# debbiemarkslab/BEAR

Hardware: AMD Instinct MI355X
Metric: k-mer contexts/sec (DM-marginal+grad h), k=13 (higher is better)
Workload: dtype f64

## Files before the change

### bear_amd/csrc/bear_hip.hip

```cpp
#include "bear_host.h"
#include "kernels_finalize.h"
#include "kernels_rows.h"
#include "kernels_sorted.h"
#include "kernels_plan.h"
#include "kernels_synth.h"
#include "kernels_refmix.h"
#include "kernels_mixplan.h"
#include "kernels_sample.h"
#include "kernels_refplan.h"

#ifdef PLN_STAMPS
#define PLN_DBG_ARG , ws->dbg
#else
#define PLN_DBG_ARG
#endif

extern "C" {

int bear_abi_version(void) { return BEAR_ABI_VERSION; }

const char *bear_strerror(int status) {
  switch (status) {
    case BEAR_OK: return "ok";
    case BEAR_ERR_INVALID_ARG: return "invalid argument (null or misaligned pointer, bad flag)";
// ... 360 lines not shown

static int plan_count_live_rows(bear_plan *p, const plan_scan &sc) {
  unsigned long long h_hist[SRT_NKEY];
  HIP_TRY(hipMemcpy(h_hist, p->hist, sizeof(h_hist), hipMemcpyDeviceToHost));
  unsigned long long live_rows = sc.heavy[1];
  for (int k = 0; k < SRT_NKEY; ++k) live_rows += h_hist[k];
  p->n_live_rows = live_rows;
  return BEAR_OK;
}

static int plan_build(const bear_ws *ws, bear_plan *p) {
  plan_scan sc;
  plan_cut cut;
  int st = plan_scan_table(ws, p, sc);
  if (st != BEAR_OK) return st;
  const char *cut_env = getenv("BEAR_PLAN_CUT");
  st = cut_env && cut_env[0] == 'h' ? cut_on_host(p, sc, cut) : cut_on_device(p, sc, cut);
  if (st != BEAR_OK) return st;
  p->tiles = cut.tiles.release();
  p->n_tiles = cut.n_tiles;
  const uint64_t stream_bytes = cut.off16 * 16 + 1024;
  const uint64_t live_bytes = p->ncol == 5 ? sizeof(uint16_t) * PLN_LIVE_STRIDE * (p->n_tiles + 1) : 0;
  st = plan_fill(ws, p, sc, stream_bytes);
  if (st == BEAR_OK && live_bytes) st = plan_live_lists(ws, p, live_bytes);
  if (st != BEAR_OK) return st;
  HIP_TRY(hipDeviceSynchronize());
  unsigned long long h_used[3] = {0, 0, 0};
  HIP_TRY(hipMemcpy(h_used, sc.cnt.get() + 3, sizeof(h_used), hipMemcpyDeviceToHost));
  for (int k = 0; k < 3; ++k) p->n_heavy[k] = h_used[k];
  st = plan_order_lists(p);
  p->n_live_rows = p->n_rows;
  if (st == BEAR_OK && p->ncol == 5) st = plan_count_live_rows(p, sc);
  p->bytes = stream_bytes + live_bytes + sizeof(pln_tile) * p->n_tiles + sizeof(pln_heavy_col) * sc.heavy[0] +
             sizeof(pln_heavy_row) * sc.heavy[1] + sizeof(uint64_t) * sc.heavy[2];
  return st;
}

int bear_plan_create(bear_ws *ws, const uint32_t *counts, uint64_t n_rows, int ncol, bear_plan **out) {
  if (!out) return BEAR_ERR_INVALID_ARG;
  *out = nullptr;
  int st = check_ws(ws);
  if (st != BEAR_OK) return st;
  if ((ncol != 4 && ncol != 5) || (n_rows && !counts) || misaligned(counts)) return BEAR_ERR_INVALID_ARG;
  plan_guard p(new (std::nothrow) bear_plan());
  if (!p) return BEAR_ERR_NOMEM;
  memset(p.get(), 0, sizeof(bear_plan));
  p->device = ws->device;
  p->ncol = ncol;
  p->n_rows = n_rows;
  p->counts = counts;
  HIP_TRY(hipMalloc(&p->hist, sizeof(unsigned long long) * PLAN_HIST_WORDS));
  HIP_TRY(hipMemset(p->hist, 0, sizeof(unsigned long long) * PLAN_HIST_WORDS));
  if (n_rows) st = plan_build(ws, p.get());
  if (st == BEAR_OK) *out = p.release();
  return st;
}

int bear_plan_destroy(bear_plan *plan) {
  if (!plan) return BEAR_OK;
  int prev = 0;
  (void)hipGetDevice(&prev);
  (void)hipSetDevice(plan->device);
  plan_free(plan);
  (void)hipSetDevice(prev);
  return BEAR_OK;
}

uint64_t bear_plan_bytes(const bear_plan *plan) { return plan ? plan->bytes : 0; }

int bear_plan_create_auto(bear_ws *ws, const uint32_t *counts, uint64_t n_rows, int *rowwise, bear_plan **out) {
  if (rowwise) *rowwise = 0;
  int st = bear_plan_create(ws, counts, n_rows, 5, out);
  if (st != BEAR_OK) return st;
  bear_plan *p = *out;
  const double cells = p->count_total[1], listed = (double)p->n_heavy[0];
  if (!(cells > 0.0) || listed * 2.0 <= cells) return BEAR_OK;
  plan_drop_sorted(p);
  plan_drop_live(p);
  p->ncol = PLAN_ROWS;
  if (rowwise) *rowwise = 1;
  return BEAR_OK;
}
static int launch_prior_rows(bear_ws *ws, const bear_plan *plan, const double *prior, const bear_params &prm, const double *theta,
                             int train_ar, double *out, double *grad_prior, hipStream_t s) {
  const int grid = grid_dense(ws, plan->n_rows);
  const double2 *lt = reinterpret_cast<const double2 *>(ws->logtab);
  const bear_step_io io = ws_io(ws, theta, BEAR_THETA_NET, out);
#define ROWS_LAUNCH(AR, GRAD) \
  hipLaunchKernelGGL((dm_prior_rows_kernel<AR, GRAD>), dim3(grid), dim3(BEAR_THREADS), 0, s, plan->counts, prior, plan->n_rows, prm, grad_prior, lt, \
                     ws->partials, io)
  BEAR_DISPATCH_2(train_ar, grad_prior, ROWS_LAUNCH);
#undef ROWS_LAUNCH
  HIP_TRY(hipGetLastError());
  return BEAR_OK;
}

uint64_t bear_plan_tile_count(const bear_plan *plan) { return plan ? plan->n_tiles : 0; }

int bear_plan_tile_info(const bear_plan *plan, uint64_t first, uint64_t count, uint64_t *row0, uint32_t *rows, uint32_t *items,
                        uint64_t *stream_offset) {
  if (!plan || first + count > plan->n_tiles || (count && (!row0 || !rows || !items || !stream_offset))) return BEAR_ERR_INVALID_ARG;
  if (!count) return BEAR_OK;
  std::vector<pln_tile> h(count);
  int prev = 0;
  (void)hipGetDevice(&prev);
  (void)hipSetDevice(plan->device);
  const hipError_t e = hipMemcpy(h.data(), plan->tiles + first, sizeof(pln_tile) * count, hipMemcpyDeviceToHost);
  (void)hipSetDevice(prev);
  HIP_TRY(e);
  for (uint64_t k = 0; k < count; ++k) {
    row0[k] = h[k].row0;
    rows[k] = h[k].rows_items >> 16;
    items[k] = h[k].rows_items & 0xffffu;
    stream_offset[k] = (uint64_t)h[k].off16 * 16;
  }
  return BEAR_OK;
}

int bear_plan_create_ref(bear_ws *ws, const uint32_t *train, const uint32_t *ref, uint64_t n_rows, bear_plan **out) {
  if (!out) return BEAR_ERR_INVALID_ARG;
  *out = nullptr;
  if ((n_rows && !ref) || misaligned(ref)) return BEAR_ERR_INVALID_ARG;
  bear_plan *created = nullptr;
  int st = bear_plan_create(ws, train, n_rows, 4, &created);
  if (st != BEAR_OK) return st;
  plan_guard p(created);
  p->ref = ref;
  if (p->count_total[1] > 0.0 && (double)p->n_heavy[0] * 2.0 > p->count_total[1]) {
    plan_drop_sorted(p.get());
    p->rows_ref = 1;
    *out = p.release();
    return BEAR_OK;
  }
  HIP_TRY(hipMalloc(&p->hist0_base, sizeof(unsigned long long) * 72));
  unsigned long long *d_meta = p->hist0_base;
  HIP_TRY(hipMemset(d_meta, 0, sizeof(unsigned long long) * 72));
  HIP_TRY(hipMalloc(&p->sum0, sizeof(double)));
  HIP_TRY(hipMemset(p->sum0, 0, sizeof(double)));
  unsigned long long h_meta[72];
  memset(h_meta, 0, sizeof(h_meta));
  const int grid = grid_capped((n_rows + 1023) / 1024, (uint64_t)ws->num_cu * 8);
  if (n_rows) {
    hipLaunchKernelGGL(rpl_build_kernel, dim3(grid), dim3(256), 0, 0, train, ref, n_rows, 0, d_meta, d_meta + 32, d_meta + 64, p->sum0,
                       static_cast<rpl_item *>(nullptr), static_cast<uint32_t *>(nullptr));
    HIP_TRY(hipGetLastError());
    HIP_TRY(hipMemcpy(h_meta, d_meta, sizeof(h_meta), hipMemcpyDeviceToHost));
  }
  unsigned long long run = 0, cur[RPL_NKEY];
  for (int k = 0; k < RPL_NKEY; ++k) {
    cur[k] = run;
    run += h_meta[k];
  }
  p->n_ref_items = run;
  p->n_heavy0 = h_meta[64];
  if (run) HIP_TRY(hipMalloc(&p->ref_items, sizeof(rpl_item) * run));
  if (p->n_heavy0) HIP_TRY(hipMalloc(&p->heavy0, sizeof(uint32_t) * p->n_heavy0));
  HIP_TRY(hipMemcpy(d_meta, cur, sizeof(cur), hipMemcpyHostToDevice));
  HIP_TRY(hipMemset(d_meta + 64, 0, sizeof(unsigned long long)));
  if (n_rows && (run || p->n_heavy0)) {
    hipLaunchKernelGGL(rpl_build_kernel, dim3(grid), dim3(256), 0, 0, train, ref, n_rows, 1, d_meta, d_meta + 32, d_meta + 64, p->sum0,
                       p->ref_items, p->heavy0);
    HIP_TRY(hipGetLastError());
  }
  HIP_TRY(hipDeviceSynchronize());
#ifdef BEAR_DET_BUILD
  for (int k = 0; k < RPL_NKEY && st == BEAR_OK; ++k) st = bear_canonical_order(p->ref_items + cur[k], h_meta[k], 16, 0);
  if (st == BEAR_OK) st = bear_canonical_order(p->heavy0, p->n_heavy0, 4, 0);
  if (st != BEAR_OK) return st;
#endif
  p->hist0 = d_meta + 32;
  p->bytes += sizeof(rpl_item) * p->n_ref_items + sizeof(uint32_t) * p->n_heavy0 + sizeof(unsigned long long) * 72;
  *out = p.release();
  return BEAR_OK;
}

static int launch_prior_plan(bear_ws *ws, const bear_plan *plan, const double *prior, uint64_t n_rows, const bear_params &prm,
                             const double *theta, int train_ar, int prior_normalized, double *out, hipStream_t s) {
  const int grid = grid_plan(ws, plan->n_tiles);
  const double2 *lt = reinterpret_cast<const double2 *>(ws->logtab);
  const bear_step_io io = ws_io(ws, theta, BEAR_THETA_NET, out);
  if (train_ar)
    hipLaunchKernelGGL((dm_prior_plan_kernel<true, true>), dim3(grid), dim3(PLN_THREADS), sizeof(pln_lds_n), s, prior, n_rows, prm,
                       plan_view(plan), lt, ws->partials, io PLN_DBG_ARG);
  else if (prior_normalized)
    hipLaunchKernelGGL((dm_prior_plan_kernel<true, false>), dim3(grid), dim3(PLN_THREADS), sizeof(pln_lds_n), s, prior, n_rows, prm,
                       plan_view(plan), lt, ws->partials, io PLN_DBG_ARG);
  else
    hipLaunchKernelGGL((dm_prior_plan_kernel<false, false>), dim3(grid), dim3(PLN_THREADS), sizeof(pln_lds_n), s, prior, n_rows, prm,
                       plan_view(plan), lt, ws->partials, io PLN_DBG_ARG);
  HIP_TRY(hipGetLastError());
  return BEAR_OK;
}

int bear_dm_prior_plan_f64(bear_ws *ws, const bear_plan *plan, const uint32_t *counts, const double *prior,
                           uint64_t n_rows, double h_signed, double eps, int train_ar, int prior_normalized,
                           double *out, void *stream) {
  int st = check_ws(ws);
  if (st != BEAR_OK) return st;
  if (!plan || !out || (n_rows && (!counts || !prior))) return BEAR_ERR_INVALID_ARG;
  if (check_plan_step(ws, plan, counts, n_rows, 5, true) != BEAR_OK || misaligned(prior) || misaligned8(out)) return BEAR_ERR_INVALID_ARG;
  const bear_params prm = params_net(h_signed, eps);
  if (plan_is_rows(plan)) return launch_prior_rows(ws, plan, prior, prm, nullptr, train_ar, out, nullptr, static_cast<hipStream_t>(stream));
  return launch_prior_plan(ws, plan, prior, n_rows, prm, nullptr, train_ar, prior_normalized, out, static_cast<hipStream_t>(stream));
}

int launch_prior_plan_grad(bear_ws *ws, const bear_plan *plan, const double *prior, const bear_params &prm,
                                  const double *theta, int train_ar, int prior_normalized, double *out, double *grad_prior,
                                  hipStream_t s) {
  const int grid = grid_plan(ws, plan->n_tiles);
  const double2 *lt = reinterpret_cast<const double2 *>(ws->logtab);
  const pln_view pv = plan_view(plan);
  const bear_step_io io = ws_io(ws, theta, BEAR_THETA_NET, out);
  if (train_ar)
    hipLaunchKernelGGL((dm_prior_plan_grad_kernel<true, true>), dim3(grid), dim3(PLN_THREADS), sizeof(pln_lds_g), s, prior, prm, pv, lt,
                       grad_prior, ws->partials, io);
  else if (prior_normalized)
    hipLaunchKernelGGL(dm_prior_plan_grad_inplace_kernel, dim3(grid), dim3(PLN_THREADS), sizeof(pln_lds_gi), s, prior, prm, pv, lt,
                       grad_prior, ws->partials, io);
  else
    hipLaunchKernelGGL((dm_prior_plan_grad_kernel<false, false>), dim3(grid), dim3(PLN_THREADS), sizeof(pln_lds_g), s, prior, prm, pv, lt,
                       grad_prior, ws->partials, io);
  HIP_TRY(hipGetLastError());
  auto fixup_grid = [&](uint64_t nh) { return grid_capped((nh + 255) / 256, (uint64_t)ws->num_cu * 8); };
#define FIXUP(NORM, AR, ROWS, N) \
  hipLaunchKernelGGL((dm_prior_grad_fixup_kernel<NORM, AR, ROWS>), dim3(fixup_grid(N)), dim3(256), 0, s, prior, prm, pv, lt, grad_prior, io)
  if (pv.n_heavy_row && !train_ar) {
    if (prior_normalized) FIXUP(true, false, true, pv.n_heavy_row);
    else FIXUP(false, false, true, pv.n_heavy_row);
  }
  if (pv.n_heavy_col) {
    if (train_ar) FIXUP(true, true, false, pv.n_heavy_col);
    else if (prior_normalized) FIXUP(true, false, false, pv.n_heavy_col);
    else FIXUP(false, false, false, pv.n_heavy_col);
  }
#undef FIXUP
  HIP_TRY(hipGetLastError());
  return BEAR_OK;
}

int bear_dm_prior_plan_grad_f64(bear_ws *ws, const bear_plan *plan, const uint32_t *counts, const double *prior,
                                uint64_t n_rows, double h_signed, double eps, int train_ar, int prior_normalized,
                                double *out, double *grad_prior, void *stream) {
  int st = check_ws(ws);
  if (st != BEAR_OK) return st;
  if (!plan || !out || !grad_prior || (n_rows && (!counts || !prior))) return BEAR_ERR_INVALID_ARG;
  if (check_plan_step(ws, plan, counts, n_rows, 5, true) != BEAR_OK) return BEAR_ERR_INVALID_ARG;
  if (misaligned(prior) || misaligned(grad_prior) || misaligned8(out)) return BEAR_ERR_INVALID_ARG;
  const bear_params prm = params_net(h_signed, eps);
  if (plan_is_rows(plan)) return launch_prior_rows(ws, plan, prior, prm, nullptr, train_ar, out, grad_prior, static_cast<hipStream_t>(stream));
  return launch_prior_plan_grad(ws, plan, prior, prm, nullptr, train_ar, prior_normalized, out, grad_prior,
                                static_cast<hipStream_t>(stream));
}

int bear_dm_prior_plan_dev_f64(bear_ws *ws, const bear_plan *plan, const uint32_t *counts, const double *prior, uint64_t n_rows,
                               const double *h_signed_dev, double eps, int train_ar, int prior_normalized, double *out,
                               double *grad_prior, void *stream) {
  int st = check_ws(ws);
  if (st != BEAR_OK) return st;
  if (!plan || !out || !h_signed_dev || (n_rows && (!counts || !prior))) return BEAR_ERR_INVALID_ARG;
  if (check_plan_step(ws, plan, counts, n_rows, 5, true) != BEAR_OK) return BEAR_ERR_INVALID_ARG;
  if (misaligned(prior) || misaligned(grad_prior) || misaligned8(out)) return BEAR_ERR_INVALID_ARG;
  hipStream_t s = static_cast<hipStream_t>(stream);
  const bear_params only_eps = params_eps(eps);
  if (plan_is_rows(plan)) return launch_prior_rows(ws, plan, prior, only_eps, h_signed_dev, train_ar, out, grad_prior, s);
  if (grad_prior) return launch_prior_plan_grad(ws, plan, prior, only_eps, h_signed_dev, train_ar, prior_normalized, out, grad_prior, s);
  return launch_prior_plan(ws, plan, prior, n_rows, only_eps, h_signed_dev, train_ar, prior_normalized, out, s);
}

int bear_dm_refmix_plan_grad_f64(bear_ws *ws, const bear_plan *plan, const uint32_t *counts, const double *net_rows,
                                 const double *ref_rows, uint64_t n_rows, const double *h_signed_dev, const double *tau_signed_dev,
                                 const double *net_weight_signed_dev, double eps, int train_ar, double *out, double *grad_net_rows,
                                 void *stream) {
  int st = check_ws(ws);
  if (st != BEAR_OK) return st;
  if (!plan || !out || !h_signed_dev || !tau_signed_dev || !net_weight_signed_dev) return BEAR_ERR_INVALID_ARG;
  if (n_rows && (!counts || !net_rows || !ref_rows || !grad_net_rows)) return BEAR_ERR_INVALID_ARG;
  if (check_plan_step(ws, plan, counts, n_rows, 5) != BEAR_OK) return BEAR_ERR_INVALID_ARG;
  if (misaligned(net_rows) || misaligned(ref_rows) || misaligned(grad_net_rows) || misaligned8(out) || misaligned8(h_signed_dev) ||
      misaligned8(tau_signed_dev) || misaligned8(net_weight_signed_dev) || !(eps >= 0.0))
    return BEAR_ERR_INVALID_ARG;
  hipStream_t s = static_cast<hipStream_t>(stream);
  const int grid = grid_plan(ws, plan->n_tiles);
  const double2 *lt = reinterpret_cast<const double2 *>(ws->logtab);
  const pln_view pv = plan_view(plan);
  const bear_step_io io = ws_io(ws, nullptr, BEAR_THETA_REF, out);
#define MIX_LAUNCH(AR)                                                                                                            \
  hipLaunchKernelGGL(dm_refmix_plan_grad_kernel<AR>, dim3(grid), dim3(PLN_THREADS), sizeof(pln_lds_g), s, net_rows, ref_rows, \
                     h_signed_dev, tau_signed_dev, net_weight_signed_dev, eps, pv, lt, grad_net_rows, ws->partials, io)
  BEAR_DISPATCH_1(train_ar, MIX_LAUNCH);
#undef MIX_LAUNCH
  HIP_TRY(hipGetLastError());
  if (pv.n_heavy_col + pv.n_heavy_row) {
    const uint64_t nh = pv.n_heavy_col + pv.n_heavy_row;
    const int g2 = grid_capped((nh + 255) / 256, (uint64_t)ws->num_cu * 4);
#define MIX_FIXUP(AR)                                                                                                      \
  hipLaunchKernelGGL(dm_refmix_fixup_kernel<AR>, dim3(g2), dim3(256), 0, s, net_rows, ref_rows, h_signed_dev, tau_signed_dev, \
                     net_weight_signed_dev, eps, pv, lt, grad_net_rows)
    BEAR_DISPATCH_1(train_ar, MIX_FIXUP);
#undef MIX_FIXUP
    HIP_TRY(hipGetLastError());
  }
  return BEAR_OK;
}


static int launch_ref_plan(bear_ws *ws, const bear_plan *plan, const uint32_t *ref, uint64_t n_rows, const bear_params &prm,
                           const double *theta, int train_ar, double *out, hipStream_t s, const bear_apply_io &apply = NO_APPLY) {
  const double2 *lt = reinterpret_cast<const double2 *>(ws->logtab);
  const bear_step_io io = ws_io(ws, theta, BEAR_THETA_REF, out);
  int grid;
  if (plan->rows_ref) {
    if (plan->ref != ref) return BEAR_ERR_INVALID_ARG;
    grid = grid_dense(ws, n_rows);
#define REF_ROWS(AR) \
  hipLaunchKernelGGL(dm_ref_rows_kernel<AR>, dim3(grid), dim3(BEAR_THREADS), 0, s, plan->counts, ref, n_rows, prm, lt, ws->partials, io, apply)
    BEAR_DISPATCH_1(train_ar, REF_ROWS);
#undef REF_ROWS
  } else if (plan->ref) {
    if (plan->ref != ref) return BEAR_ERR_INVALID_ARG;
    rpl_view rv;
    rv.items = plan->ref_items;
    rv.n_items = plan->n_ref_items;
    rv.hist0 = plan->hist0;
    rv.heavy0 = plan->heavy0;
    rv.n_heavy0 = plan->n_heavy0;
    rv.sum0 = plan->sum0;
    const uint64_t units = (plan->n_ref_items + 63) / 64, want = (units + 3) / 4 + 2, cap = (uint64_t)ws->num_cu * (units > 131072 ? 6 : 4);
    grid = grid_capped(want, cap);
#define REF_ITEMS(AR) \
  hipLaunchKernelGGL(dm_ref_items_kernel<AR>, dim3(grid), dim3(256), 0, s, prm, rv, plan_view(plan), lt, ws->partials, io, apply)
    BEAR_DISPATCH_1(train_ar, REF_ITEMS);
#undef REF_ITEMS
  } else {
    grid = grid_plan(ws, plan->n_tiles);
#define REF_PLAN(AR)                                                                                                                     \
  hipLaunchKernelGGL(dm_ref_plan_kernel<AR>, dim3(grid), dim3(PLN_THREADS), sizeof(pln_lds_r), s, ref, n_rows, prm, plan_view(plan), lt, \
                     ws->partials, io, apply)
    BEAR_DISPATCH_1(train_ar, REF_PLAN);
#undef REF_PLAN
  }
  HIP_TRY(hipGetLastError());
  return BEAR_OK;
}

int bear_dm_ref_plan_f64(bear_ws *ws, const bear_plan *plan, const uint32_t *train, const uint32_t *ref,
                         uint64_t n_rows, double h_signed, double tau_signed, double nu_signed, double eps,
                         int train_ar, double *out, void *stream) {
  int st = check_ws(ws);
  if (st != BEAR_OK) return st;
  if (!plan || !out || (n_rows && (!train || !ref))) return BEAR_ERR_INVALID_ARG;
  if (check_plan_step(ws, plan, train, n_rows, 4) != BEAR_OK || misaligned(ref) || misaligned8(out)) return BEAR_ERR_INVALID_ARG;
  return launch_ref_plan(ws, plan, ref, n_rows, params_ref(h_signed, tau_signed, nu_signed, eps), nullptr, train_ar, out,
                         static_cast<hipStream_t>(stream));
}

static int ref_reduce(bear_ws *ws, const bear_plan *plan, const uint32_t *train, const uint32_t *ref, uint64_t n_rows, const double *theta,
                      double eps, int train_ar, double *packed, hipStream_t s, const bear_apply_io &apply) {
  int st = check_ws(ws);
  if (st != BEAR_OK) return st;
  if (!plan || !packed || !theta || !n_rows || !train || !ref) return BEAR_ERR_INVALID_ARG;
  if (check_plan_step(ws, plan, train, n_rows, 4) != BEAR_OK || misaligned(ref) || misaligned8(packed)) return BEAR_ERR_INVALID_ARG;
  return launch_ref_plan(ws, plan, ref, n_rows, params_eps(eps), theta, train_ar, packed, s, apply);
}

int bear_ref_train_reduce_f64(bear_ws *ws, const bear_plan *plan, const uint32_t *train, const uint32_t *ref, uint64_t n_rows,
                              const double *theta, double eps, int train_ar, double *packed, void *stream) {
  return ref_reduce(ws, plan, train, ref, n_rows, theta, eps, train_ar, packed, static_cast<hipStream_t>(stream), NO_APPLY);
}

int bear_ref_train_step_f64(bear_ws *ws, const bear_plan *plan, const uint32_t *train, const uint32_t *ref, uint64_t n_rows,
                            double *theta, double *adam_m, double *adam_v, double *adam_t, double eps, int train_ar,
                            double learning_rate, double scale, double *out, double *loss_buf, uint64_t loss_cap, void *stream) {
  if (!adam_m || !adam_v || !adam_t) return BEAR_ERR_INVALID_ARG;
  hipStream_t s = static_cast<hipStream_t>(stream);
  if (two_launch_step()) {
    int st = ref_reduce(ws, plan, train, ref, n_rows, theta, eps, train_ar, out, s, NO_APPLY);
    if (st != BEAR_OK) return st;
    return launch_train_apply(theta, 3, out, adam_m, adam_v, adam_t, learning_rate, scale, train_ar, loss_buf, loss_cap, s);
  }
  return ref_reduce(ws, plan, train, ref, n_rows, theta, eps, train_ar, out, s,
                    make_apply(theta, 3, adam_m, adam_v, adam_t, learning_rate, scale, train_ar, loss_buf, loss_cap));
}

int bear_dm_items_f64(bear_ws *ws, const double *x, const uint32_t *c, uint64_t n, int path, double *D, double *P,
                      void *stream) {
  int st = check_ws(ws);
  if (st != BEAR_OK) return st;
  if (n == 0) return BEAR_OK;
  if (!x || !c || !D || !P || path < 0 || path > 2) return BEAR_ERR_INVALID_ARG;
  uint64_t blocks = (n + 255) / 256;
  if (blocks > 0x7fffffffull) return BEAR_ERR_INVALID_ARG;
  hipLaunchKernelGGL(dm_items_kernel, dim3((unsigned)blocks), dim3(256), 0, static_cast<hipStream_t>(stream), x, c, n, path,
                     reinterpret_cast<const double2 *>(ws->logtab), D, P);
  HIP_TRY(hipGetLastError());
  return BEAR_OK;
}

int bear_plan_count_total(const bear_plan *plan, double *total, double *bound) {
  if (!plan) return BEAR_ERR_INVALID_ARG;
  for (int k = 0; k < 3; ++k) {
    if (total) total[k] = plan->count_total[k];
    if (bound) bound[k] = plan->count_bound[k];
  }
  return BEAR_OK;
}

int bear_plan_set_count_bound(bear_plan *plan, const double *bound) {
  if (!plan || !bound) return BEAR_ERR_INVALID_ARG;
  for (int k = 0; k < 3; ++k)
    if (!(bound[k] >= plan->count_total[k]) || !(bound[k] < 0x1p50)) return BEAR_ERR_INVALID_ARG;
  for (int k = 0; k < 3; ++k) plan->count_bound[k] = bound[k];
  return BEAR_OK;
}

static int refmix_grid(const bear_ws *ws, uint64_t n_rows) { return grid_capped((n_rows + RMX_THREADS - 1) / RMX_THREADS, ws_blocks(ws, 2)); }

int bear_ref_mix_forward_f64(bear_ws *ws, const double *net_rows, const double *ref_rows, uint64_t n_rows, const double *tau_signed,
                             const double *net_weight_signed, double *prior, void *stream) {
  int st = check_ws(ws);
  if (st != BEAR_OK) return st;
  if (!tau_signed || !net_weight_signed || misaligned8(tau_signed) || misaligned8(net_weight_signed)) return BEAR_ERR_INVALID_ARG;
  if (n_rows == 0) return BEAR_OK;
  if (!net_rows || !ref_rows || !prior || misaligned(net_rows) || misaligned(ref_rows) || misaligned(prior)) return BEAR_ERR_INVALID_ARG;
  hipLaunchKernelGGL(ref_mix_forward_kernel, dim3(refmix_grid(ws, n_rows)), dim3(RMX_THREADS), 0, static_cast<hipStream_t>(stream),
                     net_rows, ref_rows, tau_signed, net_weight_signed, n_rows, prior);
  HIP_TRY(hipGetLastError());
  return BEAR_OK;
}

int bear_ref_mix_backward_f64(bear_ws *ws, const double *net_rows, const double *ref_rows, const double *grad_prior, uint64_t n_rows,
                              const double *tau_signed, const double *net_weight_signed, double *grad_net_rows, double *grad_scalars,
                              void *stream) {
  int st = check_ws(ws);
  if (st != BEAR_OK) return st;
  if (!tau_signed || !net_weight_signed || !grad_scalars || misaligned8(tau_signed) || misaligned8(net_weight_signed) ||
      misaligned8(grad_scalars))
    return BEAR_ERR_INVALID_ARG;
  hipStream_t s = static_cast<hipStream_t>(stream);
  if (n_rows == 0) {
    HIP_TRY(hipMemsetAsync(grad_scalars, 0, 2 * sizeof(double), s));
    return BEAR_OK;
  }
  if (!net_rows || !ref_rows || !grad_prior || !grad_net_rows || misaligned(net_rows) || misaligned(ref_rows) ||
      misaligned(grad_prior) || misaligned(grad_net_rows))
    return BEAR_ERR_INVALID_ARG;
  hipLaunchKernelGGL(ref_mix_backward_kernel, dim3(refmix_grid(ws, n_rows)), dim3(RMX_THREADS), 0, s, net_rows, ref_rows, grad_prior,
                     tau_signed, net_weight_signed, n_rows, grad_net_rows, ws->partials, ws_arrival(ws), grad_scalars);
  HIP_TRY(hipGetLastError());
  return BEAR_OK;
}

int bear_debug_read_timing(bear_ws *ws, unsigned long long *host, int n_words) {
  if (!ws || !host) return BEAR_ERR_INVALID_ARG;
  HIP_TRY(hipDeviceSynchronize());
  HIP_TRY(hipMemcpy(host, ws->dbg, sizeof(unsigned long long) * (size_t)n_words, hipMemcpyDeviceToHost));
  return BEAR_OK;
}

int bear_debug_occupancy(int which) {
  int nb = -1;
  hipError_t e = which == 0
      ? hipOccupancyMaxActiveBlocksPerMultiprocessor(&nb, dm_prior_sorted_kernel<0>, SRT_THREADS, sizeof(srt_lds_n))
      : hipOccupancyMaxActiveBlocksPerMultiprocessor(&nb, dm_ref_sorted_kernel, SRT_THREADS, sizeof(srt_lds_r));
  return e != hipSuccess ? -1000 - (int)e : nb;
}

int bear_log_gamma_f64(const double *conc, uint64_t n, uint64_t n_samples, uint64_t seed, double *out, void *stream) {
  if (n == 0 || n_samples == 0) return BEAR_OK;
  if (!conc || !out) return BEAR_ERR_INVALID_ARG;
  if (n_samples > (~0ull) / n) return BEAR_ERR_INVALID_ARG;
  const uint64_t total = n * n_samples;
  uint64_t blocks = (total + SMP_THREADS - 1) / SMP_THREADS;
  if (blocks > 65536) blocks = 65536;
  hipLaunchKernelGGL(log_gamma_kernel, dim3((unsigned)blocks), dim3(SMP_THREADS), 0, static_cast<hipStream_t>(stream), conc, n,
                     n_samples, seed, out);
  HIP_TRY(hipGetLastError());
  return BEAR_OK;
}

static int logdir_sample_launch(const uint32_t *counts, const double *prior, uint64_t n_rows, int width, const double *h,
                                int n_h, int with_ar, const double *van, int n_van, int mc_samples, int map, uint64_t seed,
// ... 80 lines not shown
```

### bear_amd/csrc/bear_host.h

```cpp
#pragma once
#include <hip/hip_runtime.h>
#include <math.h>
#include <stdint.h>
#include <stdlib.h>
#include <string.h>

#include <initializer_list>
#include <memory>
#include <new>
#include <vector>

#include "bear_common.h"
#include "bear_dev.h"
#include "bear_levels.h"
#include "plan_common.h"

#define BEAR_INTERNAL __attribute__((visibility("hidden")))

static inline int check_ws(const bear_ws *ws) {
  if (!ws) return BEAR_ERR_INVALID_ARG;
  int dev = -1;
  if (hipGetDevice(&dev) != hipSuccess) return BEAR_ERR_NO_DEVICE;
  if (dev != ws->device) return BEAR_ERR_WRONG_DEVICE;
  return BEAR_OK;
// ... 5 lines not shown

#define BEAR_DISPATCH_2(a, b, F) \
  do {                           \
    if (a) {                     \
      if (b) F(true, true);      \
      else F(true, false);       \
    } else {                     \
      if (b) F(false, true);     \
      else F(false, false);      \
    }                            \
  } while (0)

#define BEAR_DISPATCH_1(a, F) \
  do {                        \
    if (a) F(true);           \
    else F(false);            \
  } while (0)

#define BEAR_DISPATCH_W(width, launch) \
  do {                                 \
    if ((width) == 21) {               \
      constexpr int W = 21;            \
      launch;                          \
    } else {                           \
      constexpr int W = 5;             \
      launch;                          \
    }                                  \
  } while (0)

static inline bear_params params_eps(double eps) {
  bear_params prm;
  memset(&prm, 0, sizeof(prm));
  prm.eps = eps;
  return prm;
}
static inline bear_params params_net(double h_signed, double eps) {
  bear_params prm = params_eps(eps);
  prm.inv_h = 1.0 / exp(h_signed);
  return prm;
}
static inline bear_params params_ref(double h_signed, double tau_signed, double nu_signed, double eps) {
  bear_params prm = params_net(h_signed, eps);
  const double tau = exp(tau_signed), nw = exp(nu_signed);
  prm.E = exp(-tau);
  prm.tauE = tau * prm.E;
  prm.tau = tau;
  prm.V = 1.0 / (nw + 1.0);
  prm.nw = nw;
  return prm;
}

static inline int grid_capped(uint64_t work, uint64_t cap) {
  const uint64_t g = work < cap ? work : cap;
  return g < 1 ? 1 : (int)g;
}
static inline uint64_t ws_blocks(const bear_ws *ws, int per_cu) {
  const uint64_t g = (uint64_t)ws->num_cu * per_cu;
  return g > (uint64_t)ws->max_blocks ? (uint64_t)ws->max_blocks : g;
}
static inline int wide_grid(const bear_ws *ws, uint64_t n_rows, uint64_t tile, int per_cu) {
  return grid_capped((n_rows + tile - 1) / tile, ws_blocks(ws, per_cu));
}

static inline int grid_plan(const bear_ws *ws, uint64_t n_tiles) { return grid_capped(n_tiles, ws_blocks(ws, PLN_BLOCKS_PER_CU)); }

#define BEAR_KFN(...) reinterpret_cast<const void *>(__VA_ARGS__)
static inline int allow_dynamic_lds(std::initializer_list<const void *> kernels, size_t bytes) {
  for (const void *fn : kernels) HIP_TRY(hipFuncSetAttribute(fn, hipFuncAttributeMaxDynamicSharedMemorySize, (int)bytes));
  return BEAR_OK;
}

static inline bear_arrival ws_arrival(bear_ws *ws) {
  if (++ws->epoch == 0u) ws->epoch = 1u;
  return bear_arrival{ws->arrive, ws->epoch};
}

static inline bear_step_io ws_io(bear_ws *ws, const double *theta, int kind, double *out) {
  const bear_arrival a = ws_arrival(ws);
  bear_step_io io;
  io.theta = theta;
  io.kind = kind;
  io.epoch = a.epoch;
  io.out = out;
  io.arrive_word = a.word;
  return io;
}

static inline bool bear_deterministic() {
#ifdef BEAR_DET_BUILD
  return true;
#else
  const char *e = getenv("BEAR_AMD_DETERMINISTIC");
  return e && e[0] && e[0] != '0';
#endif
}

static const bear_apply_io NO_APPLY = {};

static inline bear_apply_io make_apply(double *theta, int n_theta, double *adam_m, double *adam_v, double *adam_t, double learning_rate,
                                       double scale, int train_ar, double *loss_buf, uint64_t loss_cap) {
  bear_apply_io A;
  A.theta = theta;
  A.m = adam_m;
  A.v = adam_v;
  A.t_state = adam_t;
  A.loss_buf = loss_buf;
  A.loss_cap = (unsigned long long)loss_cap;
  A.lr = learning_rate;
  A.scale = scale;
  A.n_theta = n_theta;
  A.train_ar = train_ar;
  return A;
}

static inline bool two_launch_step() {
  const char *e = getenv("BEAR_AMD_TWO_LAUNCH_STEP");
  return e && e[0] && e[0] != '0';
}

struct rpl_item;
struct bear_plan {
  int device;
  int ncol;
  uint64_t n_rows;
  const uint32_t *counts;
  pln_tile *tiles;
  unsigned char *stream;
  pln_heavy_col *heavy_col;
  pln_heavy_row *heavy_row;
  uint64_t *heavy_stop;
  unsigned long long *hist;
  uint16_t *live;
  uint64_t n_tiles;
  uint64_t n_heavy[3];
  int rows_ref;
  uint64_t n_live_rows;
  double count_total[3];
  double count_bound[3];
  uint64_t bytes;
  bear_level_dev cnn_levels[CNN_MAX_LAG];
  int n_cnn_levels, cnn_lag, cnn_fw;
  bear_window_dev cnn_win[CNN_MAX_LAG + 1][CNN_MAX_WIN];
  int n_cnn_win[CNN_MAX_LAG + 1];
  int n_cnn_windows;
  const uint64_t *cnn_codes;
  uint16_t *live2;
  pln_tile *tiles_p, *tiles_u;
  uint64_t n_tiles_p, n_tiles_u;
  const uint64_t *pair_codes;
  int pair_lag;
  const uint32_t *ref;
  rpl_item *ref_items;
  uint64_t n_ref_items, n_heavy0;
  unsigned long long *hist0;
  unsigned long long *hist0_base;
  uint32_t *heavy0;
  double *sum0;
};

static inline pln_view plan_view(const bear_plan *p) {
  pln_view v;
  v.tiles = p->tiles;
  v.stream = p->stream;
  v.heavy_col = p->heavy_col;
  v.heavy_row = p->heavy_row;
  v.heavy_stop = p->heavy_stop;
  v.hist = p->hist;
  v.hist_big = p->hist + 2 * SRT_NKEY;
  v.big_in_hist = 1;
  v.live = p->live;
  v.live2 = p->live2;
  v.subset = 0;
  v.n_tiles = p->n_tiles;
  v.n_heavy_col = p->n_heavy[0];
  v.n_heavy_row = p->n_heavy[1];
  v.n_heavy_stop = p->n_heavy[2];
  return v;
}

#define PLAN_ROWS 15
static inline bool plan_is_rows(const bear_plan *p) { return p->ncol == PLAN_ROWS; }
static inline int check_plan_step(const bear_ws *ws, const bear_plan *plan, const uint32_t *counts, uint64_t n_rows, int ncol,
                                  bool or_rows = false) {
  if (plan->ncol != ncol && !(or_rows && plan_is_rows(plan))) return BEAR_ERR_INVALID_ARG;
  if (plan->counts != counts || plan->n_rows != n_rows || plan->device != ws->device) return BEAR_ERR_INVALID_ARG;
  return BEAR_OK;
}

BEAR_INTERNAL int linear_ws_setup(bear_ws *ws);
BEAR_INTERNAL int cnn_ws_setup(bear_ws *ws);
BEAR_INTERNAL int eval_ws_setup(bear_ws *ws);
BEAR_INTERNAL void plan_unpair(bear_plan *plan);
BEAR_INTERNAL void plan_drop_cnn_levels(bear_plan *plan);

extern "C" {
BEAR_INTERNAL int launch_prior_plan_grad(bear_ws *ws, const bear_plan *plan, const double *prior, const bear_params &prm,
                                         const double *theta, int train_ar, int prior_normalized, double *out, double *grad_prior,
                                         hipStream_t s);
BEAR_INTERNAL int launch_train_apply(double *theta, int n_theta, const double *packed, double *adam_m, double *adam_v, double *adam_t,
                                     double learning_rate, double scale, int train_ar, double *loss_buf, uint64_t loss_cap, hipStream_t s);
}
```

### bear_amd/csrc/kernels_refplan.h

```cpp
#pragma once
#include "kernels_plan.h"

#define RPL_NKEY 32
#define RPL_HEAVY_KEY 24

struct rpl_item {
  uint32_t c, rb;
  double R;
};
static_assert(sizeof(rpl_item) == 16, "one 16-byte lane load per record");

struct rpl_view {
  const rpl_item *items;
  uint64_t n_items;
  const unsigned long long *hist0;
  const uint32_t *heavy0;
  uint64_t n_heavy0;
  const double *sum0;
};

__global__ __launch_bounds__(256) void rpl_build_kernel(const uint32_t *__restrict__ train, const uint32_t *__restrict__ ref, uint64_t n_rows,
                                                        int fill, unsigned long long *__restrict__ bucket,
                                                        unsigned long long *__restrict__ hist0, unsigned long long *__restrict__ n_heavy0,
                                                        double *__restrict__ sum0, rpl_item *__restrict__ items,
                                                        uint32_t *__restrict__ heavy0) {
  constexpr int RPT = 4;
  __shared__ uint32_t s_bucket[RPL_NKEY], s_hist0[RPL_NKEY];
  __shared__ unsigned long long s_at[RPL_NKEY];
  __shared__ double s_sum;
  const uint32_t tid = threadIdx.x;
  const uint64_t per_block = (n_rows + gridDim.x - 1) / gridDim.x;
  const uint64_t r_begin = (uint64_t)blockIdx.x * per_block, r_end = r_begin + per_block < n_rows ? r_begin + per_block : n_rows;
  for (uint64_t base = r_begin; base < r_end; base += 256u * RPT) {
    if (tid < RPL_NKEY) s_bucket[tid] = s_hist0[tid] = 0u;
    if (tid == 0) s_sum = 0.0;
    __syncthreads();
    uint32_t c[RPT][4], rb[RPT][4], rank[RPT][4];
    double R[RPT];
    double my_sum = 0.0;
#pragma unroll
    for (int k = 0; k < RPT; ++k) {
      const uint64_t row = base + tid + 256u * k;
      R[k] = -1.0;
#pragma unroll
      for (int b = 0; b < 4; ++b) c[k][b] = rb[k][b] = rank[k][b] = 0u;
      if (row < r_end) {
        uint64_t rs = 0;
#pragma unroll
        for (int b = 0; b < 4; ++b) {
          c[k][b] = train[row * 5 + b];
          rb[k][b] = ref[row * 5 + b];
          rs += rb[k][b];
        }
        R[k] = (double)rs;
#pragma unroll
        for (int b = 0; b < 4; ++b) {
          if (c[k][b] == 0u) continue;
          if (rs == 0) {
            my_sum += (double)c[k][b];
            if (c[k][b] <= SRT_CL) {
              if (!fill) atomicAdd(&s_hist0[c[k][b] - 1], 1u);
            } else if (fill) {
              heavy0[atomicAdd(n_heavy0, 1ull)] = c[k][b];
            } else {
              atomicAdd(n_heavy0, 1ull);
            }
          } else {
            const uint32_t key = (c[k][b] > SRT_CL ? SRT_CL + 1u : c[k][b]) - 1u;
            rank[k][b] = atomicAdd(&s_bucket[key], 1u);
          }
        }
      }
    }
    if (!fill && my_sum != 0.0) atomicAdd(&s_sum, my_sum);
    __syncthreads();
    if (tid < RPL_NKEY && !fill) {
      if (s_bucket[tid]) atomicAdd(&bucket[tid], (unsigned long long)s_bucket[tid]);
      if (s_hist0[tid]) atomicAdd(&hist0[tid], (unsigned long long)s_hist0[tid]);
    }
    if (!fill && tid == 0 && s_sum != 0.0) atomicAdd(sum0, s_sum);
    if (fill) {
      if (tid < RPL_NKEY) s_at[tid] = s_bucket[tid] ? atomicAdd(&bucket[tid], (unsigned long long)s_bucket[tid]) : 0ull;
      __syncthreads();
#pragma unroll
      for (int k = 0; k < RPT; ++k) {
        if (!(R[k] > 0.0)) continue;
#pragma unroll
        for (int b = 0; b < 4; ++b) {
          if (c[k][b] == 0u) continue;
          const uint32_t key = (c[k][b] > SRT_CL ? SRT_CL + 1u : c[k][b]) - 1u;
          rpl_item it;
          it.c = c[k][b];
          it.rb = rb[k][b];
          it.R = R[k];
          items[s_at[key] + rank[k][b]] = it;
        }
      }
    }
    __syncthreads();
  }
}

template <bool AR>
__global__ __launch_bounds__(256) void dm_ref_items_kernel(bear_params prm_arg, rpl_view rv, pln_view pv, const double2 *__restrict__ logtab_g,
                                                           double *__restrict__ partials, const bear_step_io io, const bear_apply_io apply) {
  __shared__ double2 s_log[BEAR_LOGTAB_N];
  const bear_params prm = bear_params_of(prm_arg, io);
  const uint32_t tid = threadIdx.x, lane = tid & 63u;
  const double u = prm.inv_h, eps = prm.eps;
  const double A = u + 5.0 * eps;
  const double x4 = prm.nw * prm.V * u + eps;
  const double VU = prm.V * u;
  const double tau = prm.tau;
  const double w2c = tau * (eps + 0.25 * VU);
  const double nwV = prm.nw * prm.V;
  double acc[4] = {0.0, 0.0, 0.0, 0.0};
  if (tid < BEAR_LOGTAB_N) s_log[tid] = logtab_g[tid];
  __syncthreads();
  auto alpha_from = [&](double rb, double R) {
    const double dev = __builtin_fma(rb + eps, bear_rcp(R), -0.25);
    return __builtin_fma(__builtin_fma(prm.E, dev, 0.25), VU, eps);
  };
  auto accumulate = [&](double x, double m, const bear_dp &o) {
    const double w1 = eps - x, P = m * o.P;
    acc[0] = __builtin_fma(m, o.D, acc[0]);
    acc[1] = __builtin_fma(w1, P, acc[1]);
    acc[2] = __builtin_fma(__builtin_fma(-tau, x, w2c), P, acc[2]);
    acc[3] = __builtin_fma(nwV * w1, P, acc[3]);
  };
  auto accumulate_ar = [&](double rb, double R, double c) {
    const double dev = __builtin_fma(rb + eps, bear_rcp(R), -0.25);
    const double f = __builtin_fma(prm.E, dev, 0.25) * prm.V;
    const double p = f + eps;
    const double dLdf = c * bear_rcp(p);
    acc[0] = __builtin_fma(c, bear_log_tab(p, s_log), acc[0]);
    acc[2] = __builtin_fma(dLdf, -prm.tauE * dev * prm.V, acc[2]);
    acc[3] = __builtin_fma(dLdf, -nwV * f, acc[3]);
  };
  const uint64_t n_units = (rv.n_items + 63u) >> 6;
  const uint64_t wave_g = ((uint64_t)blockIdx.x * 256u + tid) >> 6, n_waves = ((uint64_t)gridDim.x * 256u) >> 6;
  for (uint64_t un = wave_g; un < n_units; un += n_waves) {
    const uint64_t i = un * 64u + lane;
    rpl_item it;
    it.c = 0u;
    it.rb = 0u;
    it.R = 1.0;
    if (i < rv.n_items) it = rv.items[i];
    const double R = it.R + 4.0 * eps;
    if (AR) {
      if (it.c) accumulate_ar((double)it.rb, R, (double)it.c);
      continue;
    }
    const bool heavy = it.c > SRT_CL;
    const uint32_t cc = heavy ? SRT_CL + 1u : it.c;
    const uint32_t occ = (un + 1u) * 64u <= rv.n_items ? 64u : (uint32_t)(rv.n_items - un * 64u);
    const uint32_t cmin = occ == 64u ? (uint32_t)__builtin_amdgcn_readlane((int)cc, 0) : 0u;
    const uint32_t cmax = (uint32_t)__builtin_amdgcn_readlane((int)cc, (int)(occ - 1u));
    const double x[1] = {alpha_from((double)it.rb, R)};
    const uint32_t ci[1] = {heavy ? 0u : it.c};
    bear_dp o[1];
    srt_light<1>(x, ci, cmin > SRT_CL ? SRT_CL : cmin, cmax > SRT_CL ? SRT_CL : cmax, s_log, o);
    if (__builtin_amdgcn_ballot_w64(heavy)) {
      if (heavy) o[0] = srt_general_fast(x[0], (double)it.c, s_log);
    }
    if (it.c) accumulate(x[0], 1.0, o[0]);
  }
  const uint64_t gtid = (uint64_t)blockIdx.x * 256u + tid, gsz = (uint64_t)gridDim.x * 256u;
  const double R0 = 4.0 * eps;
  if (AR) {
    if (gtid == 0) accumulate_ar(0.0, R0, rv.sum0[0]);
    const double f4 = nwV, p4 = f4 + eps;
    double c4sum = 0.0;
    if (blockIdx.x == 0 && tid < SRT_CL) c4sum = (double)(tid + 1) * (double)pv.hist[SRT_NKEY + tid];
    for (uint64_t i = gtid; i < pv.n_heavy_stop; i += gsz) c4sum += (double)pv.heavy_stop[i];
    acc[0] = __builtin_fma(c4sum, bear_log_tab(p4, s_log), acc[0]);
    acc[3] = __builtin_fma(c4sum * bear_rcp(p4), nwV * (1.0 - f4), acc[3]);
    __syncthreads();
    block_finish<4>(acc, partials, io, apply);
    return;
  }
  const double x0 = alpha_from(0.0, R0);
  if (blockIdx.x == 0 && tid < SRT_CL) {
    const double m = (double)rv.hist0[tid];
    if (m != 0.0) accumulate(x0, m, srt_general_fast(x0, (double)(tid + 1), s_log));
  }
  for (uint64_t i = gtid; i < rv.n_heavy0; i += gsz) accumulate(x0, 1.0, srt_general_fast(x0, (double)rv.heavy0[i], s_log));
  for (uint64_t i = gtid; i < pv.n_heavy_row; i += gsz) {
    const double n = pv.heavy_row[i].n;
    if (pln_in_big_hist(pv, n)) continue;
    const bear_dp o = srt_general_fast(A, n, s_log);
    acc[0] -= o.D;
    acc[1] = __builtin_fma(u, o.P, acc[1]);
  }
  pln_big_totals(pv, A, u, gtid, gsz, s_log, acc[0], acc[1]);
  for (uint64_t i = gtid; i < pv.n_heavy_stop; i += gsz) {
    const bear_dp o = srt_general_fast(x4, (double)pv.heavy_stop[i], s_log);
    acc[0] += o.D;
    acc[1] = __builtin_fma(eps - x4, o.P, acc[1]);
    acc[3] = __builtin_fma(VU * nwV, o.P, acc[3]);
  }
  if (blockIdx.x == 1 % gridDim.x && tid < SRT_CL) {
    const double mn = (double)pv.hist[tid], m4 = (double)pv.hist[SRT_NKEY + tid];
    const bear_dp on = srt_general_fast(A, (double)(tid + 1), s_log), o4 = srt_general_fast(x4, (double)(tid + 1), s_log);
    acc[0] -= mn * on.D;
    acc[1] = __builtin_fma(u * mn, on.P, acc[1]);
    const double P4 = m4 * o4.P;
    acc[0] += m4 * o4.D;
    acc[1] = __builtin_fma(eps - x4, P4, acc[1]);
    acc[3] = __builtin_fma(VU * nwV, P4, acc[3]);
  }
  __syncthreads();
  block_finish<4>(acc, partials, io, apply);
}
```

Measured before the change: 141.2 billion.

## Collapse uniform sorted spans of ref items into single weighted evaluations

The ref item array is now always sorted canonically within each key bucket, so light items form runs of identical records. The kernel checks each 64-record span by comparing its first and last items. When they match, it evaluates the span once with weight 64 instead of processing 64 lanes. Spans that do not match fall back to per-unit processing, and heavy items past the light prefix are handled as before. The cost is a host-side canonical sort that now runs in every build, plus a changed grid-sizing heuristic. The first-equals-last check assumes full ordering within the span, which only holds if sort ties make identical records contiguous.

New measurement: 141.2 billion. Within noise of the previous version (-0.0%).

```diff
diff --git a/bear_amd/csrc/bear_hip.hip b/bear_amd/csrc/bear_hip.hip
--- a/bear_amd/csrc/bear_hip.hip
+++ b/bear_amd/csrc/bear_hip.hip
@@ -536,6 +536,7 @@
     run += h_meta[k];
   }
   p->n_ref_items = run;
+  p->n_ref_light = cur[RPL_HEAVY_KEY];
   p->n_heavy0 = h_meta[64];
   if (run) HIP_TRY(hipMalloc(&p->ref_items, sizeof(rpl_item) * run));
   if (p->n_heavy0) HIP_TRY(hipMalloc(&p->heavy0, sizeof(uint32_t) * p->n_heavy0));
@@ -547,11 +548,11 @@
     HIP_TRY(hipGetLastError());
   }
   HIP_TRY(hipDeviceSynchronize());
+  for (int k = 0; k < RPL_NKEY && st == BEAR_OK; ++k) st = bear_canonical_order(p->ref_items + cur[k], h_meta[k], 16, 0);
 #ifdef BEAR_DET_BUILD
-  for (int k = 0; k < RPL_NKEY && st == BEAR_OK; ++k) st = bear_canonical_order(p->ref_items + cur[k], h_meta[k], 16, 0);
   if (st == BEAR_OK) st = bear_canonical_order(p->heavy0, p->n_heavy0, 4, 0);
-  if (st != BEAR_OK) return st;
 #endif
+  if (st != BEAR_OK) return st;
   p->hist0 = d_meta + 32;
   p->bytes += sizeof(rpl_item) * p->n_ref_items + sizeof(uint32_t) * p->n_heavy0 + sizeof(unsigned long long) * 72;
   *out = p.release();
@@ -709,8 +710,9 @@
     rv.heavy0 = plan->heavy0;
     rv.n_heavy0 = plan->n_heavy0;
     rv.sum0 = plan->sum0;
-    const uint64_t units = (plan->n_ref_items + 63) / 64, want = (units + 3) / 4 + 2, cap = (uint64_t)ws->num_cu * (units > 131072 ? 6 : 4);
-    grid = grid_capped(want, cap);
+    rv.n_span_items = plan->n_ref_light / RPL_SPAN * RPL_SPAN;
+    const uint64_t passes = (rv.n_span_items / RPL_SPAN + 63) / 64, units = (plan->n_ref_items - rv.n_span_items + 63) / 64;
+    grid = grid_capped((std::max(passes, units) + 3) / 4 + 2, ws_blocks(ws, RPL_BLOCKS_PER_CU));
 #define REF_ITEMS(AR) \
   hipLaunchKernelGGL(dm_ref_items_kernel<AR>, dim3(grid), dim3(256), 0, s, prm, rv, plan_view(plan), lt, ws->partials, io, apply)
     BEAR_DISPATCH_1(train_ar, REF_ITEMS);
diff --git a/bear_amd/csrc/bear_host.h b/bear_amd/csrc/bear_host.h
--- a/bear_amd/csrc/bear_host.h
+++ b/bear_amd/csrc/bear_host.h
@@ -181,6 +181,7 @@
   const uint32_t *ref;
   rpl_item *ref_items;
   uint64_t n_ref_items, n_heavy0;
+  uint64_t n_ref_light;
   unsigned long long *hist0;
   unsigned long long *hist0_base;
   uint32_t *heavy0;
diff --git a/bear_amd/csrc/kernels_refplan.h b/bear_amd/csrc/kernels_refplan.h
--- a/bear_amd/csrc/kernels_refplan.h
+++ b/bear_amd/csrc/kernels_refplan.h
@@ -3,6 +3,13 @@
 
 #define RPL_NKEY 32
 #define RPL_HEAVY_KEY 24
+#ifndef RPL_SPAN
+#define RPL_SPAN 64
+#endif
+#ifndef RPL_BLOCKS_PER_CU
+#define RPL_BLOCKS_PER_CU 4
+#endif
+static_assert(RPL_SPAN >= 64 && RPL_SPAN % 64 == 0, "a span is walked in units of 64 records");
 
 struct rpl_item {
   uint32_t c, rb;
@@ -17,6 +24,7 @@
   const uint32_t *heavy0;
   uint64_t n_heavy0;
   const double *sum0;
+  uint64_t n_span_items;
 };
 
 __global__ __launch_bounds__(256) void rpl_build_kernel(const uint32_t *__restrict__ train, const uint32_t *__restrict__ ref, uint64_t n_rows,
@@ -137,34 +145,64 @@
     acc[2] = __builtin_fma(dLdf, -prm.tauE * dev * prm.V, acc[2]);
     acc[3] = __builtin_fma(dLdf, -nwV * f, acc[3]);
   };
-  const uint64_t n_units = (rv.n_items + 63u) >> 6;
-  const uint64_t wave_g = ((uint64_t)blockIdx.x * 256u + tid) >> 6, n_waves = ((uint64_t)gridDim.x * 256u) >> 6;
-  for (uint64_t un = wave_g; un < n_units; un += n_waves) {
-    const uint64_t i = un * 64u + lane;
+  auto unit = [&](uint64_t i0, uint32_t occ) {
     rpl_item it;
     it.c = 0u;
     it.rb = 0u;
     it.R = 1.0;
-    if (i < rv.n_items) it = rv.items[i];
+    if (lane < occ) it = rv.items[i0 + lane];
     const double R = it.R + 4.0 * eps;
     if (AR) {
       if (it.c) accumulate_ar((double)it.rb, R, (double)it.c);
-      continue;
+      return;
     }
     const bool heavy = it.c > SRT_CL;
     const uint32_t cc = heavy ? SRT_CL + 1u : it.c;
-    const uint32_t occ = (un + 1u) * 64u <= rv.n_items ? 64u : (uint32_t)(rv.n_items - un * 64u);
-    const uint32_t cmin = occ == 64u ? (uint32_t)__builtin_amdgcn_readlane((int)cc, 0) : 0u;
+    const uint32_t c0 = (uint32_t)__builtin_amdgcn_readlane((int)cc, 0);
     const uint32_t cmax = (uint32_t)__builtin_amdgcn_readlane((int)cc, (int)(occ - 1u));
     const double x[1] = {alpha_from((double)it.rb, R)};
     const uint32_t ci[1] = {heavy ? 0u : it.c};
-    bear_dp o[1];
-    srt_light<1>(x, ci, cmin > SRT_CL ? SRT_CL : cmin, cmax > SRT_CL ? SRT_CL : cmax, s_log, o);
+    bear_dp o[1] = {bear_dp{0.0, 0.0}};
+    if (c0 <= SRT_CL) srt_light<1>(x, ci, occ == 64u ? c0 : 0u, cmax > SRT_CL ? SRT_CL : cmax, s_log, o);
     if (__builtin_amdgcn_ballot_w64(heavy)) {
       if (heavy) o[0] = srt_general_fast(x[0], (double)it.c, s_log);
     }
     if (it.c) accumulate(x[0], 1.0, o[0]);
-  }
+  };
+  const uint64_t n_spans = rv.n_span_items / RPL_SPAN, n_passes = (n_spans + 63u) >> 6;
+  const uint64_t wave_g = ((uint64_t)blockIdx.x * 256u + tid) >> 6, n_waves = ((uint64_t)gridDim.x * 256u) >> 6;
+  for (uint64_t ps = wave_g; ps < n_passes; ps += n_waves) {
+    const uint64_t sp = ps + (uint64_t)lane * n_passes;
+    const bool have = sp < n_spans;
+    rpl_item a, b;
+    a.c = 0u;
+    a.rb = 0u;
+    a.R = 1.0;
+    b = a;
+    if (have) {
+      a = rv.items[sp * RPL_SPAN];
+      b = rv.items[sp * RPL_SPAN + (RPL_SPAN - 1u)];
+    }
+    const bool same = have && a.c == b.c && a.rb == b.rb && __double_as_longlong(a.R) == __double_as_longlong(b.R) && a.c <= SRT_CL;
+    const double R = a.R + 4.0 * eps;
+    if (AR) {
+      if (same) accumulate_ar((double)a.rb, R, (double)a.c * (double)RPL_SPAN);
+    } else {
+      const double x[1] = {alpha_from((double)a.rb, R)};
+      const uint32_t ci[1] = {same ? a.c : 0u};
+      bear_dp o[1] = {bear_dp{0.0, 0.0}};
+      const uint64_t any = __builtin_amdgcn_ballot_w64(same);
+      if (any) srt_light<1>(x, ci, 0u, (uint32_t)__builtin_amdgcn_readlane((int)ci[0], 63 - __builtin_clzll(any)), s_log, o);
+      if (same) accumulate(x[0], (double)RPL_SPAN, o[0]);
+    }
+    for (uint64_t todo = __builtin_amdgcn_ballot_w64(have && !same); todo; todo &= todo - 1u) {
+      const uint64_t i0 = (ps + (uint64_t)__builtin_ctzll(todo) * n_passes) * RPL_SPAN;
+      for (uint32_t k = 0; k < RPL_SPAN; k += 64u) unit(i0 + k, 64u);
+    }
+  }
+  const uint64_t n_units = (rv.n_items + 63u) >> 6;
+  for (uint64_t un = rv.n_span_items / 64u + wave_g; un < n_units; un += n_waves)
+    unit(un * 64u, (un + 1u) * 64u <= rv.n_items ? 64u : (uint32_t)(rv.n_items - un * 64u));
   const uint64_t gtid = (uint64_t)blockIdx.x * 256u + tid, gsz = (uint64_t)gridDim.x * 256u;
   const double R0 = 4.0 * eps;
   if (AR) {
```
